# xarray-contrib/xeofs

Measured on AMD Instinct MI355X. Metric: EOF randomized-SVD GB/s (algorithmic: 16 passes x n x p x 4 B per fit / fit time), higher is better.
Workload: dtype f32 data, split-fp16 MFMA (f16x3+f16x3), f32 accumulate

## Files before the change

xeofs_amd/csrc/eofx_abi.hip:

```cpp
#include <chrono>
#include "eofx_hfft.hpp"
#include "eofx_kernels.hpp"
#include "eofx_fit.hpp"
#include "eofx_gram.hpp"
#include "eofx_axb_dma.hpp"
#include "eofx_hosteig.hpp"
#include "eofx_hostla.hpp"
#include "eofx_lag.hpp"
#include "eofx_gw.hpp"
#include "eofx_spca.hpp"
#include "eofx_lagcov.hpp"
#include "eofx_lowpass.hpp"
#include "eofx_orderpos.hpp"
#include "eofx_colquad.hpp"
#include "eofx_pairmin.hpp"
#include "eofx_spectral.hpp"
#include "eofx_pcmul.hpp"
#include "eofx_viewcov.hpp"
#include "eofx_lrfill.hpp"
#include "eofx_plans.hpp"
#include "eofx_sketch.hpp"
#include "eofx_hilbert_host.hpp"
#include "eofx_gwplan.hpp"
#ifndef EOFX_AXB_DMA_DEFAULT
// ... 663 lines not shown
    if (ctx->axb_planes_bytes < need) {
      HIPCHK(hipStreamSynchronize(ctx->stream));
      if (ctx->axb_planes) (void)hipFree(ctx->axb_planes);
      ctx->axb_planes = nullptr;
      ctx->axb_planes_bytes = 0;
      if (hipMalloc((void**)&ctx->axb_planes, need) != hipSuccess) {
        (void)hipGetLastError();
        ctx->axb_planes = nullptr;
        dma = false;
      } else {
        ctx->axb_planes_bytes = need;
      }
    }
  }
  const int64_t pairs_all = K_all / AXB_KG;
  if (dma) {
    hipLaunchKernelGGL(axb_bsplit_kernel, dim3((unsigned)((K_all + 31) / 32), ncb), dim3(256), 0, ctx->stream, Y, L, L, K_all, bmax,
                       ctx->axb_planes);
    KCHK();
  }
  const int* const no_act = nullptr;
  for (int i = 0; i < tiles.n; ++i) {
    const ColTile& t = tiles.t[i];
    const dim3 grid(gx, t.count);
#define EOFX_AXB_ARGS(B, LDB) \
  grid, dim3(256), 0, ctx->stream, raw, ld, (int)rows, cols, aff, aff_ld, B, LDB, out, L, rows_pad, K, plan.kps, plan.S, rt, t.col_base, a_scale, bmax
    if (dma) {
      if (t.width == 64) {
        if (masked) hipLaunchKernelGGL((axb_f16_dma_kernel<4, 0, true>), EOFX_AXB_ARGS(ctx->axb_planes, pairs_all), act);
        else hipLaunchKernelGGL((axb_f16_dma_kernel<4, 0, false>), EOFX_AXB_ARGS(ctx->axb_planes, pairs_all), no_act);
      } else {
        if (masked) hipLaunchKernelGGL((axb_f16_dma_kernel<2, 0, true>), EOFX_AXB_ARGS(ctx->axb_planes, pairs_all), act);
        else hipLaunchKernelGGL((axb_f16_dma_kernel<2, 0, false>), EOFX_AXB_ARGS(ctx->axb_planes, pairs_all), no_act);
      }
    } else if (t.width == 64) {
      if (masked) hipLaunchKernelGGL((axb_f16_kernel<4, 0, true>), EOFX_AXB_ARGS(Y, L), act);
      else hipLaunchKernelGGL(axb_f16_kernel<4>, EOFX_AXB_ARGS(Y, L));
    } else {
      if (masked) hipLaunchKernelGGL((axb_f16_kernel<2, 0, true>), EOFX_AXB_ARGS(Y, L), act);
      else hipLaunchKernelGGL(axb_f16_kernel<2>, EOFX_AXB_ARGS(Y, L));
    }
#undef EOFX_AXB_ARGS
    KCHK();
  }
  if (ctx->profile) {
    HIPCHK(hipEventRecord(ev1, ctx->stream));
    ctx->prof_events.emplace_back(ev0, ev1, 1);
    ctx->prof_flops += 2.0 * (double)K * (double)rows_pad * (double)L;
    ctx->prof_bytes += (double)K * (double)rows * 4.0 * tiles.columns();
  }
  if (plan.S > 1) {
    const int64_t count4 = rows_pad * L / 4;
    hipLaunchKernelGGL(splitk_reduce_kernel, dim3((int)std::min<int64_t>((count4 + 255) / 256, amax_out ? 2048 : 4096)), dim3(256), 0,
                       ctx->stream, out, W, count4, plan.S, amax_out);
    KCHK();
  }
  return EOFX_OK;
}

static int launch_gram(eofx_ctx* ctx, const float* P, int64_t rows, int L, double* G) {
  const int nb = (L + 63) / 64;
  const int nbx = gram_parts(rows, L);
  ArenaScope scope(ctx);
  ARENA(double, part, (size_t)nbx * L * L);
  hipLaunchKernelGGL(gram_mfma_kernel, dim3(nbx, nb * nb), dim3(256), 0, ctx->stream, P, rows, L, part);
  KCHK();
  const int64_t count = (int64_t)L * L;
  hipLaunchKernelGGL(f64_reduce_kernel, dim3((int)((count + 63) / 64)), dim3(256), 0, ctx->stream,
                     part, G, count, nbx);
  KCHK();
  return EOFX_OK;
}
static int launch_matmul(eofx_ctx* ctx, const float* P, int64_t rows, int L, const double* Mx, int Lo,
                         float* out, bool upper = false) {
  int KW = (int)std::min<int64_t>(round_up(L, 64), 256);
  if (L > 256) {
    static const int kw_env = std::getenv("EOFX_PMM_KW") ? atoi(std::getenv("EOFX_PMM_KW")) : 0;
    if (kw_env == 128 || kw_env == 256) KW = kw_env;
  }
  const size_t smem = (size_t)KW * PMM_LD * sizeof(double);
  if (smem > 64 * 1024)
    HIPCHK(hipFuncSetAttribute(reinterpret_cast<const void*>(panel_matmul_kernel<false>), hipFuncAttributeMaxDynamicSharedMemorySize, (int)smem));
  const int64_t units = (rows + 127) / 128;
  const int64_t gx = L <= KW ? std::min<int64_t>(units, 1024) : units;
  dim3 grid((int)std::max<int64_t>(1, gx), (Lo + 63) / 64);
  hipLaunchKernelGGL(panel_matmul_kernel<false>, grid, dim3(256), smem, ctx->stream, P, rows, L, Mx, Lo, out, KW, amax_new(ctx, out),
                     (int64_t)0, (int64_t)0, 1, (const float*)nullptr, upper ? 1 : 0);
  KCHK();
  return EOFX_OK;
}
static int launch_matmul_gen(eofx_ctx* ctx, const float* P, int64_t ldp, int64_t slab, int cpb, int64_t rows, int L, const double* Mx, int Lo,
                             const float* sub, float* out) {
  const int KW = (int)std::min<int64_t>(round_up(L, 64), 256);
  const size_t smem = (size_t)KW * PMM_LD * sizeof(double);
  if (smem > 64 * 1024)
    HIPCHK(hipFuncSetAttribute(reinterpret_cast<const void*>(panel_matmul_kernel<true>), hipFuncAttributeMaxDynamicSharedMemorySize, (int)smem));
  const int64_t units = (rows + 127) / 128;
  const int64_t gx = L <= KW ? std::min<int64_t>(units, 1024) : units;
  dim3 grid((int)std::max<int64_t>(1, gx), (Lo + 63) / 64);
  hipLaunchKernelGGL(panel_matmul_kernel<true>, grid, dim3(256), smem, ctx->stream, P, rows, L, Mx, Lo, out, KW, amax_new(ctx, out), ldp,
                     slab, cpb, sub);
  KCHK();
  return EOFX_OK;
}
static int launch_xgram(eofx_ctx* ctx, const float* Pa, int64_t lda, int La, const float* Pb, int64_t ldb, int Lb, int64_t rows, double* C) {
  const int nbx = (int)std::max<int64_t>(1, std::min<int64_t>((rows + 127) / 128, std::max<int64_t>(1, ((int64_t)32 << 20) / ((int64_t)La * Lb * 8))));
  ArenaScope scope(ctx);
  ARENA(double, part, (size_t)nbx * La * Lb);
  hipLaunchKernelGGL(xgram_mfma_kernel, dim3(nbx, (La / 64) * (Lb / 64)), dim3(256), 0, ctx->stream, Pa, lda, Pb, ldb, rows, La, Lb, part);
  KCHK();
  const int64_t count = (int64_t)La * Lb;
  hipLaunchKernelGGL(f64_reduce_kernel, dim3((int)((count + 63) / 64)), dim3(256), 0, ctx->stream, part, C, count, nbx);
  KCHK();
  return EOFX_OK;
}

static int launch_rinv(eofx_ctx* ctx, const double* G, int L, int l, double* Rinv);
static size_t matmul_nt_scratch(eofx_ctx* ctx, int64_t rows, int L, int Lo);
static int launch_matmul_nt(eofx_ctx* ctx, const float* P, int64_t rows, int L, const double* Mx, int Lo, float* out);
static int launch_cholqr(eofx_ctx* ctx, const float* P, int64_t rows, int L, int l, const double* G,
                         float* out) {
  ArenaScope scope(ctx);
  ARENA(double, Rinv, (size_t)L * L);
  CHK(launch_rinv(ctx, G, L, l, Rinv));
  return launch_matmul(ctx, P, rows, L, Rinv, L, out, true);
}

static int launch_colminmax(eofx_ctx* ctx, const float* P, int64_t rows, int L, float* mx, float* mn) {
  const int nparts = (int)std::max<int64_t>(1, std::min<int64_t>((rows + 127) / 128, 1024));
  ArenaScope scope(ctx);
  ARENA(float, pmx, (size_t)nparts * L);
  ARENA(float, pmn, (size_t)nparts * L);
  hipLaunchKernelGGL(colminmax_part_kernel, dim3(nparts, (L + 63) / 64), dim3(256), 0, ctx->stream, P,
                     rows, L, pmx, pmn);
  KCHK();
  hipLaunchKernelGGL(colminmax_final_kernel, dim3((L + 63) / 64), dim3(256), 0, ctx->stream, pmx, pmn,
                     nparts, L, mx, mn);
  KCHK();
  return EOFX_OK;
}

static int export_panel(eofx_ctx* ctx, const float* P, int64_t rows, int L, int k, const double* sign,
                        float* dst) {
  if (!dst) return EOFX_OK;
  ArenaScope scope(ctx);
  double* dsign = nullptr;
  if (sign) {
    dsign = arena_alloc<double>(ctx, k);
    if (!dsign) return set_err(ctx, EOFX_ERR_NOMEM, "arena exhausted (export sign)");
    CHK(copy_in(ctx, dsign, sign, sizeof(double) * k));
  }
  float* tmp = dst;
  const bool dev = is_device_ptr(dst);
  if (!dev) {
    tmp = arena_alloc<float>(ctx, (size_t)rows * k);
    if (!tmp) return set_err(ctx, EOFX_ERR_NOMEM, "arena exhausted (export staging)");
  }
  const int64_t total = rows * k;
  const int blocks = (int)std::min<int64_t>((total + 255) / 256, 8192);
  hipLaunchKernelGGL(panel_export_kernel, dim3(blocks), dim3(256), 0, ctx->stream, P, rows, L, k, dsign,
                     tmp);
  KCHK();
  if (!dev) {
    CHK(copy_out(ctx, dst, tmp, sizeof(float) * total));
    HIPCHK(hipStreamSynchronize(ctx->stream));
  }
  return EOFX_OK;
// ... 4614 lines not shown
```

xeofs_amd/csrc/eofx_kernels.hpp:

```cpp
#pragma once
#include <hip/hip_runtime.h>
#include <stdint.h>

#include "eofx_mfma64.hpp"
#include "eofx_plans.hpp"

namespace eofx {

typedef float f32x16 __attribute__((ext_vector_type(16)));
typedef float f32x4 __attribute__((ext_vector_type(4)));
typedef float f32x2 __attribute__((ext_vector_type(2)));

__device__ __forceinline__ void aff_split(double sh, float& hi, float& lo) {
  hi = (float)sh;
  lo = (float)(sh - (double)hi);
}
__device__ __forceinline__ float aff_map(float x, float sh_hi, float sh_lo, float scale) {
  return ((x - sh_hi) - sh_lo) * scale;
}
__device__ __forceinline__ float aff_fma(float x, float sh_hi, float s, float nls) {
  return __builtin_fmaf(x - sh_hi, s, nls);
}

__device__ __forceinline__ void amax_commit(float mx, unsigned* __restrict__ amax_out) {
  __shared__ float amax_red_[16];
#pragma unroll
  for (int o = 32; o > 0; o >>= 1) mx = fmaxf(mx, __shfl_xor(mx, o));
  if ((threadIdx.x & 63) == 0) amax_red_[threadIdx.x >> 6] = mx;
  __syncthreads();
  if (threadIdx.x == 0) {
    const int nw = (int)(blockDim.x >> 6);
    float m = amax_red_[0];
    for (int w = 1; w < nw; ++w) m = fmaxf(m, amax_red_[w]);
    if (m > 0.f) atomicMax(amax_out, __float_as_uint(m));
  }
}

constexpr int ATB_KC = 16;
constexpr int ATB_WM = 128;

template <int NB>
__global__ __launch_bounds__(256, 2) void atb_f32_kernel(const float* __restrict__ A, int64_t lda,
                                                          const float* __restrict__ B, int ldb,
                                                          float* __restrict__ C, int ldc, int64_t M,
                                                          int64_t K, int64_t k_per_split,
                                                          int col_base) {
  __shared__ __attribute__((aligned(16))) float Bs[2][ATB_KC][32 * NB];
  const int tid = threadIdx.x;
  const int lane = tid & 63;
  const int wave = tid >> 6;
  const int li = lane & 31, lh = lane >> 5;
  const int64_t m0 = (int64_t)blockIdx.x * ATB_BM + wave * ATB_WM;
  const int64_t kb = (int64_t)blockIdx.y * k_per_split;
  const int64_t ke = (kb + k_per_split < K) ? kb + k_per_split : K;
  const int nchunks = (int)((ke - kb) / ATB_KC);
  const int bcol0 = col_base + blockIdx.z * 64;

  f32x16 acc[4][NB];
#pragma unroll
  for (int j = 0; j < 4; ++j)
#pragma unroll
    for (int b = 0; b < NB; ++b)
#pragma unroll
      for (int r = 0; r < 16; ++r) acc[j][b][r] = 0.f;

  const float* Ap = A + (kb + lh) * lda + m0 + 4 * li;
  constexpr int BV = 8 * NB;
  const bool b_loader = tid < 16 * BV;
  const int brow = tid / BV, bc4 = tid % BV;
  const float* Bp = B + (kb + brow) * (int64_t)ldb + bcol0 + 4 * bc4;

  f32x4 a0[8], a1[8];
  f32x4 bn = {0.f, 0.f, 0.f, 0.f};
#define EOFX_LOAD_SLAB(areg, chunk)                                                              \
  do {                                                                                           \
    if (b_loader) bn = *reinterpret_cast<const f32x4*>(Bp + (int64_t)(chunk) * ATB_KC * ldb);   \
    const float* pa_ = Ap + (int64_t)(chunk) * ATB_KC * lda;                                     \
    _Pragma("unroll") for (int i = 0; i < 8; ++i) areg[i] =                                      \
        __builtin_nontemporal_load(reinterpret_cast<const f32x4*>(pa_ + (int64_t)(2 * i) * lda)); \
  } while (0)
#define EOFX_COMPUTE_SLAB(areg, buf)                                                             \
  do {                                                                                           \
    _Pragma("unroll") for (int i = 0; i < 8; ++i) {                                              \
      float b_[NB];                                                                              \
      _Pragma("unroll") for (int q = 0; q < NB; ++q) b_[q] = Bs[buf][2 * i + lh][32 * q + li];   \
      _Pragma("unroll") for (int j = 0; j < 4; ++j) _Pragma("unroll") for (int q = 0; q < NB; ++q) \
          acc[j][q] = __builtin_amdgcn_mfma_f32_32x32x2f32(areg[i][j], b_[q], acc[j][q], 0, 0, 0); \
    }                                                                                            \
  } while (0)
#define EOFX_STORE_B(buf)                                                                        \
  do {                                                                                           \
    if (b_loader) *reinterpret_cast<f32x4*>(&Bs[buf][brow][4 * bc4]) = bn;                       \
  } while (0)

// ... 803 lines not shown
    __syncthreads();
    for (int c = 0; c < nchunks; c += 2) {
      EOFX_LOAD_SLAB(a1, c + 1);
      __builtin_amdgcn_sched_barrier(0);
      EOFX_COMPUTE_SLAB(a0, 0);
      EOFX_STORE_B(1);
      __syncthreads();
      const int c2 = (c + 2 < nchunks) ? c + 2 : c + 1;
      EOFX_LOAD_SLAB(a0, c2);
      __builtin_amdgcn_sched_barrier(0);
      EOFX_COMPUTE_SLAB(a1, 1);
      EOFX_STORE_B(0);
      __syncthreads();
    }
  }
#undef EOFX_LOAD_SLAB
#undef EOFX_COMPUTE_SLAB
#undef EOFX_STORE_B

#pragma unroll
  for (int t = 0; t < 4; ++t)
#pragma unroll
    for (int q = 0; q < NT; ++q)
#pragma unroll
      for (int r = 0; r < 4; ++r) {
        const int i = kq + 4 * r;
        const int64_t m = m0 + 4 * i + t;
        const int64_t o = m * ldc + bcol0 + 16 * q + c16;
        if (Cd)
          Cd[(int64_t)blockIdx.y * M * ldc + o] = acc[t][q][r];
        else
          C[o] = (float)acc[t][q][r];
      }
}

__global__ __launch_bounds__(256) void splitk_reduce_f64_kernel(const double* __restrict__ part, float* __restrict__ out,
                                                                int64_t count, int splits) {
  const int64_t stride = (int64_t)gridDim.x * blockDim.x;
  for (int64_t i = (int64_t)blockIdx.x * blockDim.x + threadIdx.x; i < count; i += stride) {
    double s = 0.0;
    for (int k = 0; k < splits; ++k) s += part[(int64_t)k * count + i];
    out[i] = (float)s;
  }
}

__global__ __launch_bounds__(256) void splitk_reduce_kernel(const float* __restrict__ part,
                                                            float* __restrict__ out,
                                                            int64_t count4, int splits,
                                                            unsigned* __restrict__ amax_out = nullptr) {
  const int64_t stride = (int64_t)gridDim.x * blockDim.x;
  float mx = 0.f;
  for (int64_t i = (int64_t)blockIdx.x * blockDim.x + threadIdx.x; i < count4; i += stride) {
    double s0 = 0, s1 = 0, s2 = 0, s3 = 0;
    for (int s = 0; s < splits; ++s) {
      const f32x4 v = reinterpret_cast<const f32x4*>(part)[(int64_t)s * count4 + i];
      s0 += v[0];
      s1 += v[1];
      s2 += v[2];
      s3 += v[3];
    }
    f32x4 o = {(float)s0, (float)s1, (float)s2, (float)s3};
    reinterpret_cast<f32x4*>(out)[i] = o;
    mx = fmaxf(mx, fmaxf(fmaxf(fabsf(o[0]), fabsf(o[1])), fmaxf(fabsf(o[2]), fabsf(o[3]))));
  }
  if (amax_out) amax_commit(mx, amax_out);
}

__global__ __launch_bounds__(256) void symmetrize_lower_kernel(float* __restrict__ C, int64_t n, int64_t ld) {
  __shared__ float T[64][65];
  const int bi = blockIdx.y, bj = blockIdx.x;
  if (bj > bi) return;
  const int tx = threadIdx.x & 63, ty = threadIdx.x >> 6;
  for (int r = ty; r < 64; r += 4) {
    const int64_t gr = (int64_t)bj * 64 + r, gc = (int64_t)bi * 64 + tx;
    T[r][tx] = (gr < n && gc < n) ? C[gr * ld + gc] : 0.f;
  }
  __syncthreads();
  for (int r = ty; r < 64; r += 4) {
    const int64_t gr = (int64_t)bi * 64 + r, gc = (int64_t)bj * 64 + tx;
    if (gr < n && gc < n && gc < gr) C[gr * ld + gc] = T[tx][r];
  }
}

__global__ __launch_bounds__(256) void gram_mfma_kernel(const float* __restrict__ P, int64_t rows, int L,
                                                         double* __restrict__ Gpart) {
  const int nb = (L + 63) / 64;
  const int bi = blockIdx.y / nb, bj = blockIdx.y % nb;
  if (bi > bj) return;
  const int wave = threadIdx.x >> 6;
  const Mfma64Lane ln = mfma64_lane();
  const int ca = 64 * bi + 4 * ln.c, cb = 64 * bj + 4 * ln.c;
  const bool same = (bi == bj);
  f64x4 acc[4][4];
  mfma64_zero(acc);
  const int64_t wstride = (int64_t)gridDim.x * 4 * 4;
  auto fetch = [&](int64_t r0, f32x4& va, f32x4& vb) {
    const int64_t r = r0 + ln.k;
    va = f32x4{0.f, 0.f, 0.f, 0.f};
    vb = va;
    if (r < rows) {
      if (ca < L) va = *reinterpret_cast<const f32x4*>(P + r * L + ca);
      if (!same && cb < L) vb = *reinterpret_cast<const f32x4*>(P + r * L + cb);
    }
    if (same) vb = va;
  };
  constexpr int GRAM_PF = 4;
  int64_t r0 = ((int64_t)blockIdx.x * 4 + wave) * 4;
  f32x4 pa[GRAM_PF], pb[GRAM_PF];
#pragma unroll
  for (int d = 0; d < GRAM_PF; ++d) fetch(r0 + d * wstride, pa[d], pb[d]);
  for (; r0 < rows; r0 += GRAM_PF * wstride) {
#pragma unroll
    for (int d = 0; d < GRAM_PF; ++d) {
      const f32x4 va = pa[d], vb = pb[d];
      fetch(r0 + (GRAM_PF + d) * wstride, pa[d], pb[d]);
      __builtin_amdgcn_sched_barrier(0);
      const double a[4] = {(double)va[0], (double)va[1], (double)va[2], (double)va[3]};
      const double b[4] = {(double)vb[0], (double)vb[1], (double)vb[2], (double)vb[3]};
      if (same)
        mfma64_step(acc, a, b, [](int x, int y) { return y >= x; });
      else
        mfma64_step(acc, a, b, Mfma64All{});
    }
  }
  __shared__ double Gs[64][65];
  for (int w = 0; w < 4; ++w) {
    if (wave == w)
      mfma64_each_interleaved(acc, [&](int x, int y) { return !(same && x > y); },
                              [&](int x, int y, int i, int j, double v) {
                                if (w == 0) {
                                  Gs[i][j] = v;
                                  if (same && x < y) Gs[j][i] = v;
                                } else {
                                  Gs[i][j] += v;
                                  if (same && x < y) Gs[j][i] += v;
                                }
                              });
    __syncthreads();
  }
  double* G = Gpart + (int64_t)blockIdx.x * (int64_t)L * L;
  for (int e = threadIdx.x; e < 64 * 64; e += 256) {
    const int i = e >> 6, j = e & 63;
    const int gi = 64 * bi + i, gj = 64 * bj + j;
    if (gi < L && gj < L) {
      G[(int64_t)gi * L + gj] = Gs[i][j];
      if (!same) G[(int64_t)gj * L + gi] = Gs[i][j];
    }
  }
}

__global__ __launch_bounds__(256) void f64_reduce_kernel(const double* __restrict__ part,
                                                         double* __restrict__ out, int64_t count,
                                                         int nparts) {
  __shared__ double red[4][64];
  const int li = threadIdx.x & 63, q = threadIdx.x >> 6;
  const int64_t i = (int64_t)blockIdx.x * 64 + li;
  double s = 0;
  if (i < count) {
#pragma unroll 4
    for (int b = q; b < nparts; b += 4) s += part[(int64_t)b * count + i];
  }
  red[q][li] = s;
  __syncthreads();
  if (q == 0 && i < count) out[i] = ((red[0][li] + red[1][li]) + red[2][li]) + red[3][li];
}

__global__ __launch_bounds__(256) void xgram_mfma_kernel(const float* __restrict__ Pa, int64_t lda, const float* __restrict__ Pb,
                                                          int64_t ldb, int64_t rows, int La, int Lb, double* __restrict__ part) {
  const int nbj = Lb / 64;
  const int bi = blockIdx.y / nbj, bj = blockIdx.y % nbj;
  const int lane = threadIdx.x & 63, wave = threadIdx.x >> 6;
  const int lc = lane & 15, lk = lane >> 4;
  const int ca = 64 * bi + 4 * lc, cb = 64 * bj + 4 * lc;
  f64x4 acc[4][4];
#pragma unroll
  for (int x = 0; x < 4; ++x)
#pragma unroll
    for (int y = 0; y < 4; ++y) acc[x][y] = f64x4{0.0, 0.0, 0.0, 0.0};
  const int64_t wstride = (int64_t)gridDim.x * 4 * 4;
  auto fetch = [&](int64_t r0, f32x4& va, f32x4& vb) {
    const int64_t r = r0 + lk;
    va = f32x4{0.f, 0.f, 0.f, 0.f};
    vb = va;
    if (r < rows) {
      va = *reinterpret_cast<const f32x4*>(Pa + r * lda + ca);
      vb = *reinterpret_cast<const f32x4*>(Pb + r * ldb + cb);
    }
  };
  constexpr int XG_PF = 4;
  int64_t r0 = ((int64_t)blockIdx.x * 4 + wave) * 4;
  f32x4 pa[XG_PF], pb[XG_PF];
#pragma unroll
  for (int d = 0; d < XG_PF; ++d) fetch(r0 + d * wstride, pa[d], pb[d]);
  for (; r0 < rows; r0 += XG_PF * wstride) {
#pragma unroll
    for (int d = 0; d < XG_PF; ++d) {
      const f32x4 va = pa[d], vb = pb[d];
      fetch(r0 + (XG_PF + d) * wstride, pa[d], pb[d]);
      __builtin_amdgcn_sched_barrier(0);
#pragma unroll
      for (int x = 0; x < 4; ++x)
#pragma unroll
        for (int y = 0; y < 4; ++y)
          acc[x][y] = __builtin_amdgcn_mfma_f64_16x16x4f64((double)va[x], (double)vb[y], acc[x][y], 0, 0, 0);
    }
  }
  __shared__ double Gs[64][65];
// ... 160 lines not shown
    const int r = i >> 6, c = i & 63;
    if (r < L && c < L) Rinv[(int64_t)r * L + c] = (r <= c && c < l && !dead[c]) ? X[r][c] : 0.0;
  }
  EOFX_RINV_T(4);
#undef EOFX_RINV_T
}

template <bool TA>
__global__ __launch_bounds__(256) void dgemm64_kernel(const double* __restrict__ A, int lda, const double* B, int ldb,
                                                       double* C, int ldc, int K, double alpha, double beta, int upper,
                                                       int64_t sA = 0, int64_t sB = 0, int64_t sC = 0) {
  __shared__ double As[16][65], Bs[16][65];
  const int bx = blockIdx.x, by = blockIdx.y;
  if (upper && by > bx) return;
  A += (int64_t)blockIdx.z * sA;
  B += (int64_t)blockIdx.z * sB;
  C += (int64_t)blockIdx.z * sC;
  const int tx = threadIdx.x & 15, ty = threadIdx.x >> 4;
  double acc[4][4];
#pragma unroll
  for (int i = 0; i < 4; ++i)
#pragma unroll
    for (int j = 0; j < 4; ++j) acc[i][j] = 0.0;
  for (int k0 = 0; k0 < K; k0 += 16) {
#pragma unroll
    for (int e = 0; e < 4; ++e) {
      const int idx = threadIdx.x + 256 * e;
      if (TA) {
        const int k = idx >> 6, m = idx & 63;
        As[k][m] = A[(int64_t)(k0 + k) * lda + 64 * by + m];
      } else {
        const int m = idx >> 4, k = idx & 15;
        As[k][m] = A[(int64_t)(64 * by + m) * lda + k0 + k];
      }
      const int kb = idx >> 6, n = idx & 63;
      Bs[kb][n] = B[(int64_t)(k0 + kb) * ldb + 64 * bx + n];
    }
    __syncthreads();
#pragma unroll
    for (int k = 0; k < 16; ++k) {
      double a[4], b[4];
#pragma unroll
      for (int i = 0; i < 4; ++i) a[i] = As[k][4 * ty + i];
#pragma unroll
      for (int j = 0; j < 4; ++j) b[j] = Bs[k][4 * tx + j];
#pragma unroll
      for (int i = 0; i < 4; ++i)
#pragma unroll
        for (int j = 0; j < 4; ++j) acc[i][j] = __builtin_fma(a[i], b[j], acc[i][j]);
    }
    __syncthreads();
  }
#pragma unroll
  for (int i = 0; i < 4; ++i)
#pragma unroll
    for (int j = 0; j < 4; ++j) {
      double* c = C + (int64_t)(64 * by + 4 * ty + i) * ldc + 64 * bx + 4 * tx + j;
      *c = beta == 0.0 ? alpha * acc[i][j] : alpha * acc[i][j] + beta * *c;
    }
}

__global__ void chol_blocked_init_kernel(const double* __restrict__ G, int L, int l, double* __restrict__ S, int Lb,
                                          double* __restrict__ d0) {
  const int64_t total = (int64_t)Lb * Lb;
  for (int64_t i = (int64_t)blockIdx.x * blockDim.x + threadIdx.x; i < total; i += (int64_t)gridDim.x * blockDim.x) {
    const int r = (int)(i / Lb), c = (int)(i % Lb);
    double v = (r == c) ? 1.0 : 0.0;
    if (r < l && c < l) v = G[(int64_t)r * L + c];
    S[i] = v;
    if (r == c) d0[r] = v;
  }
}
__global__ void chol_blocked_export_kernel(const double* __restrict__ X, int Lb, int l, double* __restrict__ Rinv, int L) {
  const int64_t total = (int64_t)L * L;
  for (int64_t i = (int64_t)blockIdx.x * blockDim.x + threadIdx.x; i < total; i += (int64_t)gridDim.x * blockDim.x) {
    const int r = (int)(i / L), c = (int)(i % L);
    Rinv[i] = (r <= c && c < l) ? X[(int64_t)r * Lb + c] : 0.0;
  }
}

constexpr int PMM_LD = 66;

template <bool GEN = false>
__global__ __launch_bounds__(256) void panel_matmul_kernel(const float* __restrict__ P,
                                                           int64_t rows, int L,
                                                           const double* __restrict__ Mx, int Lo,
                                                           float* __restrict__ out, int KW,
                                                           unsigned* __restrict__ amax_out = nullptr,
                                                           int64_t ldp = 0, int64_t slab = 0, int cpb = 1,
                                                           const float* __restrict__ sub = nullptr, int upper = 0) {
  extern __shared__ __attribute__((aligned(16))) double Ms[];
  float amx = 0.f;
  const int tid = threadIdx.x;
  const int lane = tid & 63, wave = tid >> 6;
  const int li = lane & 15, lk = lane >> 4;
  const int by = upper ? (int)(gridDim.y - 1 - blockIdx.y) : (int)blockIdx.y;
  const int c0 = by * 64;
  const int Lc_all = (L + 63) / 64;
  const int Lc = upper ? (Lc_all < by + 1 ? Lc_all : by + 1) : Lc_all;
  const int Le = L < 64 * Lc ? L : 64 * Lc;
  const int64_t ngroups = (rows + 31) / 32;
  const int64_t g0 = (int64_t)blockIdx.x * 4 + wave;
  auto stage = [&](int k0) {
    for (int i = tid; i < KW * 64; i += 256) {
      const int r = i >> 6, c = i & 63;
      Ms[r * PMM_LD + c] = (k0 + r < L && c0 + c < Lo) ? Mx[(int64_t)(k0 + r) * Lo + c0 + c] : 0.0;
    }
  };
  auto fetch = [&](bool valid, int64_t g, int kc, f32x4 (&a)[2][4]) {
#pragma unroll
    for (int t = 0; t < 2; ++t) {
      const int64_t r = 32 * g + 16 * t + li;
#pragma unroll
      for (int tt = 0; tt < 4; ++tt) {
        const int k = kc + 16 * tt + 4 * lk;
        if constexpr (GEN)
          a[t][tt] = (valid && r < rows && k < L) ? *reinterpret_cast<const f32x4*>(P + (int64_t)((k >> 6) / cpb) * slab + ((k >> 6) % cpb) * 64 + r * ldp + (k & 63))
                                                 : f32x4{0.f, 0.f, 0.f, 0.f};
        else
          a[t][tt] = (valid && r < rows && k < L) ? *reinterpret_cast<const f32x4*>(P + r * L + k)
                                                 : f32x4{0.f, 0.f, 0.f, 0.f};
      }
    }
  };
  f64x4 acc[2][4];
  auto compute = [&](int64_t g, int kc, int ms0, const f32x4 (&a)[2][4]) {
    if (kc == 0) {
#pragma unroll
      for (int t = 0; t < 2; ++t)
#pragma unroll
        for (int q = 0; q < 4; ++q) acc[t][q] = f64x4{0.0, 0.0, 0.0, 0.0};
    }
#pragma unroll
    for (int tt = 0; tt < 4; ++tt)
#pragma unroll
      for (int c = 0; c < 4; ++c) {
        double b[4];
#pragma unroll
        for (int q = 0; q < 4; ++q) b[q] = Ms[(kc - ms0 + 16 * tt + 4 * lk + c) * PMM_LD + 16 * q + li];
#pragma unroll
        for (int t = 0; t < 2; ++t)
#pragma unroll
          for (int q = 0; q < 4; ++q)
            acc[t][q] = __builtin_amdgcn_mfma_f64_16x16x4f64((double)a[t][tt][c], b[q], acc[t][q], 0, 0, 0);
      }
    if (kc + 64 >= Le) {
#pragma unroll
      for (int t = 0; t < 2; ++t)
#pragma unroll
        for (int r = 0; r < 4; ++r) {
          const int64_t row = 32 * g + 16 * t + lk + 4 * r;
          if (row >= rows) continue;
#pragma unroll
          for (int q = 0; q < 4; ++q) {
            const int col = c0 + 16 * q + li;
            if (col < Lo) {
              float o_ = (float)acc[t][q][r];
              if constexpr (GEN) {
                if (sub) o_ = (float)((double)sub[row * Lo + col] - acc[t][q][r]);
              }
              out[row * Lo + col] = o_;
              amx = fmaxf(amx, fabsf(o_));
            }
          }
        }
    }
  };
  f32x4 a0[2][4], a1[2][4];
  if (Lc * 64 <= KW) {
    stage(0);
    __syncthreads();
    const int64_t gstride = (int64_t)gridDim.x * 4;
    const int64_t nitems = g0 < ngroups ? ((ngroups - g0 + gstride - 1) / gstride) * Lc : 0;
    fetch(nitems > 0, g0, 0, a0);
    for (int64_t item = 0; item < nitems; item += 2) {
      fetch(item + 1 < nitems, g0 + ((item + 1) / Lc) * gstride, (int)((item + 1) % Lc) * 64, a1);
      __builtin_amdgcn_sched_barrier(0);
      compute(g0 + (item / Lc) * gstride, (int)(item % Lc) * 64, 0, a0);
      if (item + 1 < nitems) {
        fetch(item + 2 < nitems, g0 + ((item + 2) / Lc) * gstride, (int)((item + 2) % Lc) * 64, a0);
        __builtin_amdgcn_sched_barrier(0);
        compute(g0 + ((item + 1) / Lc) * gstride, (int)((item + 1) % Lc) * 64, 0, a1);
      }
    }
  } else {
    const bool active = g0 < ngroups;
    const int wc = KW / 64;
    fetch(active, g0, 0, a0);
    for (int w0 = 0; w0 < Lc; w0 += wc) {
      __syncthreads();
      stage(64 * w0);
      __syncthreads();
      const int we = w0 + wc < Lc ? w0 + wc : Lc;
      for (int ch = w0; ch < we; ch += 2) {
        fetch(active && ch + 1 < Lc, g0, 64 * (ch + 1), a1);
        __builtin_amdgcn_sched_barrier(0);
        if (active) compute(g0, 64 * ch, 64 * w0, a0);
        fetch(active && ch + 2 < Lc, g0, 64 * (ch + 2), a0);
        __builtin_amdgcn_sched_barrier(0);
        if (active && ch + 1 < we) compute(g0, 64 * (ch + 1), 64 * w0, a1);
      }
    }
  }
  if (amax_out) amax_commit(amx, amax_out);
}

__global__ __launch_bounds__(256) void colminmax_part_kernel(const float* __restrict__ P,
                                                             int64_t rows, int L,
                                                             float* __restrict__ pmx,
                                                             float* __restrict__ pmn) {
  __shared__ float smx[16][64], smn[16][64];
  const int tid = threadIdx.x;
  const int cq = tid & 15, rl = tid >> 4;
  const int c = blockIdx.y * 64 + 4 * cq;
  f32x4 mx = {-INFINITY, -INFINITY, -INFINITY, -INFINITY}, mn = {INFINITY, INFINITY, INFINITY, INFINITY};
  if (c < L) {
    const int64_t step = (int64_t)gridDim.x * 16;
    int64_t r = (int64_t)blockIdx.x * 16 + rl;
    for (; r + 7 * step < rows; r += 8 * step) {
      f32x4 v[8];
#pragma unroll
      for (int u = 0; u < 8; ++u) v[u] = *reinterpret_cast<const f32x4*>(P + (r + u * step) * L + c);
#pragma unroll
      for (int u = 0; u < 8; ++u)
#pragma unroll
        for (int e = 0; e < 4; ++e) {
          mx[e] = fmaxf(mx[e], v[u][e]);
          mn[e] = fminf(mn[e], v[u][e]);
        }
    }
    for (; r < rows; r += step) {
      const f32x4 v = *reinterpret_cast<const f32x4*>(P + r * L + c);
#pragma unroll
      for (int e = 0; e < 4; ++e) {
        mx[e] = fmaxf(mx[e], v[e]);
        mn[e] = fminf(mn[e], v[e]);
      }
    }
  }
#pragma unroll
  for (int e = 0; e < 4; ++e) {
    smx[rl][4 * cq + e] = mx[e];
    smn[rl][4 * cq + e] = mn[e];
  }
  __syncthreads();
  if (tid < 64 && blockIdx.y * 64 + tid < L) {
    float a = smx[0][tid], b = smn[0][tid];
    for (int q = 1; q < 16; ++q) {
      a = fmaxf(a, smx[q][tid]);
      b = fminf(b, smn[q][tid]);
    }
    pmx[(int64_t)blockIdx.x * L + blockIdx.y * 64 + tid] = a;
    pmn[(int64_t)blockIdx.x * L + blockIdx.y * 64 + tid] = b;
  }
}
__global__ __launch_bounds__(256) void colminmax_final_kernel(const float* __restrict__ pmx,
                                                              const float* __restrict__ pmn, int nparts, int L,
                                                              float* __restrict__ mx, float* __restrict__ mn) {
  __shared__ float sa[4][64], sb[4][64];
  const int li = threadIdx.x & 63, qq = threadIdx.x >> 6;
  const int c = blockIdx.x * 64 + li;
  float a = -INFINITY, b = INFINITY;
  if (c < L) {
#pragma unroll 8
    for (int q = qq; q < nparts; q += 4) {
// ... 1086 lines not shown
```

Before: 5992.

## Restructure gram and panel-matmul pipelines with branchless loads and double-buffered LDS fragments

The gram kernel is split into diagonal and off-diagonal templated paths. The diagonal path no longer loads or keeps a second operand, and scheduling barriers now order prefetches. Panel matmul does branchless zero-pointer loads and batches 16 LDS stage loads into registers. It double-buffers B fragments from LDS around each MFMA group and replaces per-item div/mod with incremental index stepping. Both kernels gain launch_bounds occupancy 2 and the panel-matmul grid cap drops to 512, which risks register spills and lower parallelism.

```diff
diff --git a/xeofs_amd/csrc/eofx_abi.hip b/xeofs_amd/csrc/eofx_abi.hip
--- a/xeofs_amd/csrc/eofx_abi.hip
+++ b/xeofs_amd/csrc/eofx_abi.hip
@@ -769,7 +769,7 @@
   if (smem > 64 * 1024)
     HIPCHK(hipFuncSetAttribute(reinterpret_cast<const void*>(panel_matmul_kernel<false>), hipFuncAttributeMaxDynamicSharedMemorySize, (int)smem));
   const int64_t units = (rows + 127) / 128;
-  const int64_t gx = L <= KW ? std::min<int64_t>(units, 1024) : units;
+  const int64_t gx = L <= KW ? std::min<int64_t>(units, 512) : units;
   dim3 grid((int)std::max<int64_t>(1, gx), (Lo + 63) / 64);
   hipLaunchKernelGGL(panel_matmul_kernel<false>, grid, dim3(256), smem, ctx->stream, P, rows, L, Mx, Lo, out, KW, amax_new(ctx, out),
                      (int64_t)0, (int64_t)0, 1, (const float*)nullptr, upper ? 1 : 0);
diff --git a/xeofs_amd/csrc/eofx_kernels.hpp b/xeofs_amd/csrc/eofx_kernels.hpp
--- a/xeofs_amd/csrc/eofx_kernels.hpp
+++ b/xeofs_amd/csrc/eofx_kernels.hpp
@@ -10,6 +10,12 @@
 typedef float f32x16 __attribute__((ext_vector_type(16)));
 typedef float f32x4 __attribute__((ext_vector_type(4)));
 typedef float f32x2 __attribute__((ext_vector_type(2)));
+
+__device__ __attribute__((aligned(16))) float zero_f32x4[4];
+__device__ __forceinline__ const f32x4* zero_or(bool ok, const float* p) {
+  return ok ? reinterpret_cast<const f32x4*>(p) : reinterpret_cast<const f32x4*>(zero_f32x4);
+}
+__device__ __forceinline__ void vm_landed() { __builtin_amdgcn_s_waitcnt(0x0F70); }
 
 __device__ __forceinline__ void aff_split(double sh, float& hi, float& lo) {
   hi = (float)sh;
@@ -979,7 +985,45 @@
   }
 }
 
-__global__ __launch_bounds__(256) void gram_mfma_kernel(const float* __restrict__ P, int64_t rows, int L,
+#ifndef GRAM_PF_DIAG
+#define GRAM_PF_DIAG 4
+#endif
+#ifndef GRAM_PF_OFF
+#define GRAM_PF_OFF 4
+#endif
+template <bool SAME, int PF>
+__device__ __forceinline__ void gram_accumulate(const float* __restrict__ P, int64_t rows, int L, int ca, int cb, int lk,
+                                                int64_t r0, int64_t wstride, f64x4 (&acc)[4][4]) {
+  const bool ina = ca < L, inb = cb < L;
+  auto fetch = [&](int64_t rr, f32x4& va, f32x4& vb) {
+    const int64_t r = rr + lk;
+    va = *zero_or(r < rows && ina, P + r * L + ca);
+    if constexpr (!SAME) vb = *zero_or(r < rows && inb, P + r * L + cb);
+  };
+  f32x4 pa[PF], pb[SAME ? 1 : PF];
+#pragma unroll
+  for (int d = 0; d < PF; ++d) {
+    fetch(r0 + d * wstride, pa[d], pb[SAME ? 0 : d]);
+    __builtin_amdgcn_sched_barrier(0);
+  }
+  for (; r0 < rows; r0 += PF * wstride) {
+#pragma unroll
+    for (int d = 0; d < PF; ++d) {
+      const f32x4 va = pa[d], vb = SAME ? va : pb[SAME ? 0 : d];
+      const double a[4] = {(double)va[0], (double)va[1], (double)va[2], (double)va[3]};
+      const double b[4] = {(double)vb[0], (double)vb[1], (double)vb[2], (double)vb[3]};
+      __builtin_amdgcn_sched_barrier(0);
+      fetch(r0 + (PF + d) * wstride, pa[d], pb[SAME ? 0 : d]);
+      __builtin_amdgcn_sched_barrier(0);
+      if constexpr (SAME)
+        mfma64_step(acc, a, b, [](int x, int y) { return y >= x; });
+      else
+        mfma64_step(acc, a, b, Mfma64All{});
+    }
+  }
+}
+
+__global__ __launch_bounds__(256, 2) void gram_mfma_kernel(const float* __restrict__ P, int64_t rows, int L,
                                                          double* __restrict__ Gpart) {
   const int nb = (L + 63) / 64;
   const int bi = blockIdx.y / nb, bj = blockIdx.y % nb;
@@ -991,35 +1035,11 @@
   f64x4 acc[4][4];
   mfma64_zero(acc);
   const int64_t wstride = (int64_t)gridDim.x * 4 * 4;
-  auto fetch = [&](int64_t r0, f32x4& va, f32x4& vb) {
-    const int64_t r = r0 + ln.k;
-    va = f32x4{0.f, 0.f, 0.f, 0.f};
-    vb = va;
-    if (r < rows) {
-      if (ca < L) va = *reinterpret_cast<const f32x4*>(P + r * L + ca);
-      if (!same && cb < L) vb = *reinterpret_cast<const f32x4*>(P + r * L + cb);
-    }
-    if (same) vb = va;
-  };
-  constexpr int GRAM_PF = 4;
-  int64_t r0 = ((int64_t)blockIdx.x * 4 + wave) * 4;
-  f32x4 pa[GRAM_PF], pb[GRAM_PF];
-#pragma unroll
-  for (int d = 0; d < GRAM_PF; ++d) fetch(r0 + d * wstride, pa[d], pb[d]);
-  for (; r0 < rows; r0 += GRAM_PF * wstride) {
-#pragma unroll
-    for (int d = 0; d < GRAM_PF; ++d) {
-      const f32x4 va = pa[d], vb = pb[d];
-      fetch(r0 + (GRAM_PF + d) * wstride, pa[d], pb[d]);
-      __builtin_amdgcn_sched_barrier(0);
-      const double a[4] = {(double)va[0], (double)va[1], (double)va[2], (double)va[3]};
-      const double b[4] = {(double)vb[0], (double)vb[1], (double)vb[2], (double)vb[3]};
-      if (same)
-        mfma64_step(acc, a, b, [](int x, int y) { return y >= x; });
-      else
-        mfma64_step(acc, a, b, Mfma64All{});
-    }
-  }
+  const int64_t r0 = ((int64_t)blockIdx.x * 4 + wave) * 4;
+  if (same)
+    gram_accumulate<true, GRAM_PF_DIAG>(P, rows, L, ca, cb, ln.k, r0, wstride, acc);
+  else
+    gram_accumulate<false, GRAM_PF_OFF>(P, rows, L, ca, cb, ln.k, r0, wstride, acc);
   __shared__ double Gs[64][65];
   for (int w = 0; w < 4; ++w) {
     if (wave == w)
@@ -1346,7 +1366,7 @@
 constexpr int PMM_LD = 66;
 
 template <bool GEN = false>
-__global__ __launch_bounds__(256) void panel_matmul_kernel(const float* __restrict__ P,
+__global__ __launch_bounds__(256, 2) void panel_matmul_kernel(const float* __restrict__ P,
                                                            int64_t rows, int L,
                                                            const double* __restrict__ Mx, int Lo,
                                                            float* __restrict__ out, int KW,
@@ -1366,9 +1386,15 @@
   const int64_t ngroups = (rows + 31) / 32;
   const int64_t g0 = (int64_t)blockIdx.x * 4 + wave;
   auto stage = [&](int k0) {
-    for (int i = tid; i < KW * 64; i += 256) {
-      const int r = i >> 6, c = i & 63;
-      Ms[r * PMM_LD + c] = (k0 + r < L && c0 + c < Lo) ? Mx[(int64_t)(k0 + r) * Lo + c0 + c] : 0.0;
+    for (int i0 = tid; i0 < KW * 64; i0 += 256 * 16) {
+      double v[16];
+#pragma unroll
+      for (int u = 0; u < 16; ++u) {
+        const int r = (i0 >> 6) + 4 * u, c = i0 & 63;
+        v[u] = *((k0 + r < L && c0 + c < Lo) ? Mx + (int64_t)(k0 + r) * Lo + c0 + c : reinterpret_cast<const double*>(zero_f32x4));
+      }
+#pragma unroll
+      for (int u = 0; u < 16; ++u) Ms[((i0 >> 6) + 4 * u) * PMM_LD + (i0 & 63)] = v[u];
     }
   };
   auto fetch = [&](bool valid, int64_t g, int kc, f32x4 (&a)[2][4]) {
@@ -1379,11 +1405,9 @@
       for (int tt = 0; tt < 4; ++tt) {
         const int k = kc + 16 * tt + 4 * lk;
         if constexpr (GEN)
-          a[t][tt] = (valid && r < rows && k < L) ? *reinterpret_cast<const f32x4*>(P + (int64_t)((k >> 6) / cpb) * slab + ((k >> 6) % cpb) * 64 + r * ldp + (k & 63))
-                                                 : f32x4{0.f, 0.f, 0.f, 0.f};
+          a[t][tt] = *zero_or(valid && r < rows && k < L, P + (int64_t)((k >> 6) / cpb) * slab + ((k >> 6) % cpb) * 64 + r * ldp + (k & 63));
         else
-          a[t][tt] = (valid && r < rows && k < L) ? *reinterpret_cast<const f32x4*>(P + r * L + k)
-                                                 : f32x4{0.f, 0.f, 0.f, 0.f};
+          a[t][tt] = *zero_or(valid && r < rows && k < L, P + r * L + k);
       }
     }
   };
@@ -1395,19 +1419,25 @@
 #pragma unroll
         for (int q = 0; q < 4; ++q) acc[t][q] = f64x4{0.0, 0.0, 0.0, 0.0};
     }
-#pragma unroll
-    for (int tt = 0; tt < 4; ++tt)
-#pragma unroll
-      for (int c = 0; c < 4; ++c) {
-        double b[4];
-#pragma unroll
-        for (int q = 0; q < 4; ++q) b[q] = Ms[(kc - ms0 + 16 * tt + 4 * lk + c) * PMM_LD + 16 * q + li];
-#pragma unroll
-        for (int t = 0; t < 2; ++t)
-#pragma unroll
-          for (int q = 0; q < 4; ++q)
-            acc[t][q] = __builtin_amdgcn_mfma_f64_16x16x4f64((double)a[t][tt][c], b[q], acc[t][q], 0, 0, 0);
-      }
+    const double* mb = Ms + (kc - ms0 + 4 * lk) * PMM_LD + li;
+    auto bfrag = [&](int s, double (&b)[4]) {
+#pragma unroll
+      for (int q = 0; q < 4; ++q) b[q] = mb[(16 * (s >> 2) + (s & 3)) * PMM_LD + 16 * q];
+    };
+    double b[2][4];
+    bfrag(0, b[0]);
+#pragma unroll
+    for (int s = 0; s < 16; ++s) {
+      if (s + 1 < 16) bfrag(s + 1, b[(s + 1) & 1]);
+      __builtin_amdgcn_sched_barrier(0);
+#pragma unroll
+      for (int t = 0; t < 2; ++t)
+#pragma unroll
+        for (int q = 0; q < 4; ++q)
+          acc[t][q] = __builtin_amdgcn_mfma_f64_16x16x4f64((double)a[t][s >> 2][s & 3], b[s & 1][q], acc[t][q], 0, 0, 0);
+      __builtin_amdgcn_sched_barrier(0);
+    }
+    vm_landed();
     if (kc + 64 >= Le) {
 #pragma unroll
       for (int t = 0; t < 2; ++t)
@@ -1436,15 +1466,29 @@
     __syncthreads();
     const int64_t gstride = (int64_t)gridDim.x * 4;
     const int64_t nitems = g0 < ngroups ? ((ngroups - g0 + gstride - 1) / gstride) * Lc : 0;
-    fetch(nitems > 0, g0, 0, a0);
+    auto next = [&](int64_t& g, int& kc) {
+      kc += 64;
+      if (kc == 64 * Lc) {
+        kc = 0;
+        g += gstride;
+      }
+    };
+    int64_t ga = g0, gb = g0;
+    int ka = 0, kb = 0;
+    fetch(nitems > 0, ga, ka, a0);
+    vm_landed();
     for (int64_t item = 0; item < nitems; item += 2) {
-      fetch(item + 1 < nitems, g0 + ((item + 1) / Lc) * gstride, (int)((item + 1) % Lc) * 64, a1);
+      gb = ga, kb = ka;
+      next(gb, kb);
+      fetch(item + 1 < nitems, gb, kb, a1);
       __builtin_amdgcn_sched_barrier(0);
-      compute(g0 + (item / Lc) * gstride, (int)(item % Lc) * 64, 0, a0);
+      compute(ga, ka, 0, a0);
       if (item + 1 < nitems) {
-        fetch(item + 2 < nitems, g0 + ((item + 2) / Lc) * gstride, (int)((item + 2) % Lc) * 64, a0);
+        ga = gb, ka = kb;
+        next(ga, ka);
+        fetch(item + 2 < nitems, ga, ka, a0);
         __builtin_amdgcn_sched_barrier(0);
-        compute(g0 + ((item + 1) / Lc) * gstride, (int)((item + 1) % Lc) * 64, 0, a1);
+        compute(gb, kb, 0, a1);
       }
     }
   } else {
```

Measured after the change: 5907. -1.4%, worse.
